# sidward14/gan-lab

Hardware: AMD Instinct MI355X
Metric: images/sec (G+D step), StyleGAN 1024^2 bs32/GPU (higher is better)
Workload: dtype f32; 1 GPU; StyleGAN res_samples=1024 FFHQ-shaped synthetic, bs=32/GPU fp32, nonsaturating + R1(lambda=10) + drift, stabilised phase, 1 D-iter + 1 G-iter; global_batch=32, per_gpu_batch=32, parallelism=single

## Files before the change

### gan_lab_amd/_lib.py

```python
import ctypes
import os
import subprocess

import torch

_HERE = os.path.dirname(os.path.abspath(__file__))
CSRC = os.path.join(_HERE, 'csrc')
SO_PATH = os.path.join(CSRC, os.path.basename(os.environ.get('GANLAB_HIP_LIB', '') or 'libganlab_hip.so'))

_c_int, _c_ll, _c_f, _c_p, _c_sz, _c_u64 = (ctypes.c_int, ctypes.c_longlong, ctypes.c_float, ctypes.c_void_p,
                                             ctypes.c_size_t, ctypes.c_uint64)
_c_d = ctypes.c_double

ACT_NONE, ACT_LRELU = 0, 1
PACK_FWD, PACK_DGRAD = 0, 1


class ConvGeom(ctypes.Structure):
    _fields_ = [('N', _c_int), ('Cin', _c_int), ('Hin', _c_int), ('Win', _c_int),
                ('Cout', _c_int), ('ks', _c_int), ('pad', _c_int), ('up', _c_int), ('pool', _c_int)]


_GP = ctypes.POINTER(ConvGeom)

# ... 42 lines not shown
    'ganlab_conv_splitk_plan': (_c_int, [_GP, _c_int]),
    'ganlab_conv_fwd_splitk_f32': (_c_int, [_c_p, _c_p, _c_p, _c_p, _GP, _c_f, _c_int, _c_f, _c_p, _c_sz, _c_p]),
    'ganlab_conv_dgrad_splitk_f32': (_c_int, [_c_p, _c_p, _c_p, _GP, _c_p, _c_sz, _c_p]),
    'ganlab_conv_dgrad_mask_supported': (_c_int, [_GP]),
    'ganlab_conv_dgrad_mask_f32': (_c_int, [_c_p, _c_p, _c_p, _c_p, _GP, _c_f, _c_p]),
    'ganlab_conv_act_bwd_fused_supported': (_c_int, [_GP]),
    'ganlab_conv_dgrad_act_f32': (_c_int, [_c_p, _c_p, _c_p, _c_p, _GP, _c_f, _c_p]),
    'ganlab_conv_fwd_mask_f32': (_c_int, [_c_p, _c_p, _c_p, _c_p, _GP, _c_f, _c_p]),
    'ganlab_conv_wgrad_act_f32': (_c_int, [_c_p, _c_p, _c_p, _c_p, _c_p, _GP, _c_f, _c_f, _c_f, _c_p, _c_sz, _c_p]),
    'ganlab_conv_wgrad_workspace': (_c_sz, [_GP]),
    'ganlab_conv_wgrad_f32': (_c_int, [_c_p, _c_p, _c_p, _GP, _c_f, _c_p, _c_sz, _c_p]),
    'ganlab_conv_s2_supported': (_c_int, [_GP]),
    'ganlab_conv_s2_pack_f32': (_c_ll, [_c_p, _c_p, _c_int, _c_int, _c_int, _c_int, _c_f, _c_p]),
    'ganlab_conv_s2_fwd_f32': (_c_int, [_c_p, _c_p, _c_p, _c_p, _GP, _c_f, _c_int, _c_f, _c_p]),
    'ganlab_conv_s2_dgrad_f32': (_c_int, [_c_p, _c_p, _c_p, _GP, _c_p]),
    'ganlab_conv_s2_wgrad_workspace': (_c_sz, [_GP]),
    'ganlab_conv_s2_wgrad_f32': (_c_int, [_c_p, _c_p, _c_p, _GP, _c_f, _c_p, _c_sz, _c_p]),
    'ganlab_conv_bf16_supported': (_c_int, [_GP]),
    'ganlab_conv_pack_bf16': (_c_ll, [_c_p, _c_p, _c_int, _c_int, _c_int, _c_f, _c_p]),
    'ganlab_conv_fwd_bf16': (_c_int, [_c_p, _c_p, _c_p, _c_p, _GP, _c_f, _c_int, _c_f, _c_p]),
    'ganlab_conv_dgrad_bf16': (_c_int, [_c_p, _c_p, _c_p, _GP, _c_p]),
    'ganlab_conv_bf16_splitk_plan': (_c_int, [_GP, _c_int]),
    'ganlab_conv_fwd_bf16_splitk': (_c_int, [_c_p, _c_p, _c_p, _c_p, _GP, _c_f, _c_int, _c_f, _c_p, _c_sz, _c_p]),
    'ganlab_conv_dgrad_bf16_splitk': (_c_int, [_c_p, _c_p, _c_p, _GP, _c_p, _c_sz, _c_p]),
    'ganlab_conv_wgrad_bf16_workspace': (_c_sz, [_GP]),
    'ganlab_conv_wgrad_bf16': (_c_int, [_c_p, _c_p, _c_p, _GP, _c_f, _c_p, _c_sz, _c_p]),
    'ganlab_conv_x3_supported': (_c_int, [_GP, _c_int]),
    'ganlab_conv_x3_pack': (_c_ll, [_c_p, _c_p, _c_int, _c_int, _c_int, _c_f, _c_p]),
    'ganlab_conv_fwd_x3': (_c_int, [_c_p, _c_p, _c_p, _c_p, _GP, _c_f, _c_int, _c_f, _c_p]),
    'ganlab_conv_dgrad_x3': (_c_int, [_c_p, _c_p, _c_p, _GP, _c_p]),
    'ganlab_conv_dgrad_mask_x3': (_c_int, [_c_p, _c_p, _c_p, _c_p, _GP, _c_f, _c_p]),
    'ganlab_conv_fwd_aff_x3': (_c_int, [_c_p, _c_p, _c_p, _c_p, _c_p, _c_p, _GP, _c_f, _c_int, _c_f, _c_p]),
    'ganlab_conv_fwd_aff_tail_x3_chunks': (_c_int, [_GP]),
    'ganlab_conv_s2_x3_supported': (_c_int, [_GP, _c_int]),
    'ganlab_conv_s2_x3_pack': (_c_ll, [_c_p, _c_p, _c_int, _c_int, _c_int, _c_f, _c_p]),
    'ganlab_conv_s2_fwd_x3': (_c_int, [_c_p, _c_p, _c_p, _c_p, _GP, _c_f, _c_int, _c_f, _c_p]),
    'ganlab_conv_s2_fwd_aff_x3': (_c_int, [_c_p, _c_p, _c_p, _c_p, _c_p, _c_p, _GP, _c_f, _c_int, _c_f, _c_p]),
    'ganlab_conv_s2_dgrad_x3': (_c_int, [_c_p, _c_p, _c_p, _GP, _c_p]),
    'ganlab_conv_s2_down_x3_supported': (_c_int, [_GP, _c_int]),
    'ganlab_conv_s2_down_x3_pack': (_c_ll, [_c_p, _c_p, _c_int, _c_int, _c_int, _c_f, _c_p]),
    'ganlab_conv_s2_down_fwd_x3': (_c_int, [_c_p, _c_p, _c_p, _c_p, _GP, _c_f, _c_int, _c_f, _c_p]),
    'ganlab_conv_s2_down_dgrad_x3': (_c_int, [_c_p, _c_p, _c_p, _GP, _c_p]),
    'ganlab_conv_wgrad_x3_supported': (_c_int, [_GP]),
    'ganlab_conv_wgrad_x3_workspace': (_c_sz, [_GP]),
    'ganlab_conv_wgrad_x3': (_c_int, [_c_p, _c_p, _c_p, _c_p, _c_p, _GP, _c_f, _c_p, _c_sz, _c_p]),
    'ganlab_conv_s2_wgrad_x3_supported': (_c_int, [_GP]),
    'ganlab_conv_s2_wgrad_x3_workspace': (_c_sz, [_GP]),
    'ganlab_conv_s2_wgrad_x3': (_c_int, [_c_p, _c_p, _c_p, _c_p, _c_p, _GP, _c_f, _c_p, _c_sz, _c_p]),
    'ganlab_conv_fwd_aff_tail_x3': (_c_int, [_c_p, _c_p, _c_p, _c_p, _c_p, _c_p, _c_p, _c_p, _c_p, _c_p, _GP, _c_f, _c_int, _c_f,
                                             _c_f, _c_p, _c_sz, _c_p]),
    'ganlab_mask_bits_supported': (_c_int, [_c_int, _c_int]),
    'ganlab_blur3x3_bits_f32': (_c_int, [_c_p, _c_p, _c_p, _c_ll, _c_int, _c_int, _c_p]),
    'ganlab_blur_act_bwd_bits_f32': (_c_int, [_c_p, _c_p, _c_p, _c_p, _c_int, _c_int, _c_int, _c_int, _c_f, _c_f,
                                              _c_p, _c_sz, _c_p]),
    'ganlab_act_bwd_blur_bits_f32': (_c_int, [_c_p, _c_p, _c_p, _c_p, _c_p, _c_p, _c_int, _c_int, _c_int, _c_int,
                                              _c_f, _c_f, _c_p, _c_sz, _c_p]),
    'ganlab_conv_fwd_blur_supported': (_c_int, [_GP, _c_p, _c_p]),
    'ganlab_conv_fwd_blur_bits_f32': (_c_int, [_c_p, _c_p, _c_p, _c_p, _c_p, _GP, _c_f, _c_f, _c_p]),
    'ganlab_conv_s2_blur_supported': (_c_int, [_GP]),
    'ganlab_conv_s2_blur_workspace': (_c_sz, [_GP]),
    'ganlab_conv_s2_fwd_blur_tail_f32': (_c_int, [_c_p, _c_p, _c_p, _c_p, _c_p, _c_p, _c_p, _c_p, _c_p, _c_p, _GP, _c_f, _c_int,
                                                  _c_f, _c_f, _c_p, _c_sz, _c_p]),
    'ganlab_conv_s2_dgrad_blur_act_bits_f32': (_c_int, [_c_p, _c_p, _c_p, _c_p, _c_p, _GP, _c_f, _c_f, _c_p, _c_sz, _c_p]),
    'ganlab_conv_dgrad_rgb_sums_supported': (_c_int, [_GP, _c_int]),
    'ganlab_conv_dgrad_rgb_sums_workspace': (_c_sz, [_GP]),
    'ganlab_conv_dgrad_rgb_sums_f32': (_c_int, [_c_p, _c_p, _c_p, _c_p, _c_p, _c_p, _GP, _c_int, _c_f, _c_f, _c_f, _c_int, _c_int,
# ... 290 lines not shown
```

### gan_lab_amd/csrc/common.h

```cpp
#pragma once
#include <hip/hip_runtime.h>
#include <stdint.h>

#include "../../include/ganlab_hip.h"

typedef float f32x4 __attribute__((ext_vector_type(4)));

static thread_local int gl_launch_status = GANLAB_OK;
extern thread_local const void* gl_last_kernel_fn;
extern thread_local unsigned gl_last_grid;
#define GL_LAUNCH_RING 16
extern thread_local const void* gl_ring_fn[GL_LAUNCH_RING];
extern thread_local unsigned gl_ring_grid[GL_LAUNCH_RING];
extern thread_local unsigned long long gl_launch_count;
#define GL_LAUNCH(k, grid, ...)                                                  \
  do {                                                                           \
    (void)hipGetLastError();                                                     \
    const dim3 gl_grid_ = (grid);                                                \
    gl_last_kernel_fn = reinterpret_cast<const void*>(k);                        \
    gl_last_grid = gl_grid_.x * gl_grid_.y * gl_grid_.z;                         \
    gl_ring_fn[gl_launch_count % GL_LAUNCH_RING] = gl_last_kernel_fn;            \
    gl_ring_grid[gl_launch_count % GL_LAUNCH_RING] = gl_last_grid;               \
    ++gl_launch_count;                                                           \
    hipLaunchKernelGGL(k, gl_grid_, __VA_ARGS__);                                \
// ... 70 lines not shown
    const float w = ci < Cin ? wp[(long long)ci * Cout_p + co] : 0.f;
    a.x += w * xv[ci].x; a.y += w * xv[ci].y; a.z += w * xv[ci].z; a.w += w * xv[ci].w;
  }
  return a;
}

struct gl_bf16x3 { __bf16 h, m, l; };
__device__ __forceinline__ gl_bf16x3 gl_split3(float v) {
  const __bf16 h = (__bf16)v;
  const float r1 = v - (float)h;
  const __bf16 m = (__bf16)r1;
  return gl_bf16x3{h, m, (__bf16)(r1 - (float)m)};
}

__device__ __forceinline__ void gl_x3_pack_position(const float* __restrict__ w9, bool flip, float scale, __bf16* __restrict__ out,
                                                    int CI, int ci, int co) {
  const int steps = CI / 32 * 9;
  const int ct = co >> 6, col = co & 63, c = ci >> 5, half = (ci >> 4) & 1, g = (ci >> 3) & 1, j = ci & 7;
#pragma unroll
  for (int t = 0; t < 9; ++t) {
    const int s = t < 8 ? (half ? 5 : 0) + (t >> 1) : 4;
    const int hi = t < 8 ? (t & 1) : half;
    const int kg = hi * 2 + g;
    float v = w9[flip ? 8 - t : t] * scale;
    asm volatile("" : "+v"(v));
    const gl_bf16x3 p = gl_split3(v);
    __bf16* base = out + (((long long)ct * steps + c * 9 + s) * (3 * 4 * 64)) * 8;
    base[((0 * 4 + kg) * 64 + col) * 8 + j] = p.h;
    base[((1 * 4 + kg) * 64 + col) * 8 + j] = p.m;
    base[((2 * 4 + kg) * 64 + col) * 8 + j] = p.l;
  }
}

__device__ __forceinline__ void gl_x3_up_pack_position(const float* __restrict__ w9, int up, float scale, __bf16* __restrict__ out,
                                                       int CI, int CO, int ci, int co) {
  const int nsteps = CI / 8;
  const bool c32 = (CO & 63) != 0;
  const int ct = c32 ? co >> 5 : co >> 6, j = ci & 7;
#pragma unroll
  for (int py = 0; py < 2; ++py)
#pragma unroll
    for (int px = 0; px < 2; ++px)
#pragma unroll
      for (int ty = 0; ty < 2; ++ty)
#pragma unroll
        for (int tx = 0; tx < 2; ++tx) {
          float v = 0.f;
#pragma unroll
          for (int ky = 0; ky < 3; ++ky)
#pragma unroll
            for (int kx = 0; kx < 3; ++kx) {
              const int ry = up ? ky : 2 - ky, rx = up ? kx : 2 - kx;
              const bool iny = py == 0 ? (ty == 0 ? ry == 0 : ry >= 1) : (ty == 0 ? ry <= 1 : ry == 2);
              const bool inx = px == 0 ? (tx == 0 ? rx == 0 : rx >= 1) : (tx == 0 ? rx <= 1 : rx == 2);
              if (iny && inx) v += w9[ky * 3 + kx];
            }
          v = v * (up ? scale : 0.25f * scale);
          asm volatile("" : "+v"(v));
          const gl_bf16x3 p = gl_split3(v);
          __bf16* base = out + (((c32 ? (long long)ct : (long long)ct * 2 + py) * nsteps + (ci >> 3)) * (3 * 4 * 128)) * 8;
          const int col = c32 ? py * 32 + (co & 31) : co & 63;
          const int kgq = ty * 2 + tx;
          base[((0 * 4 + kgq) * 128 + px * 64 + col) * 8 + j] = p.h;
          base[((1 * 4 + kgq) * 128 + px * 64 + col) * 8 + j] = p.m;
          base[((2 * 4 + kgq) * 128 + px * 64 + col) * 8 + j] = p.l;
        }
// ... 58 lines not shown
```

### gan_lab_amd/csrc/pack.hip

```cpp
#include "common.h"

namespace {

constexpr int round_up_c(int v, int m) { return (v + m - 1) / m * m; }

__global__ __launch_bounds__(256) void pack_many_kernel(const ganlab_pack_desc* __restrict__ descs, int n_desc) {
  int lo = 0, hi = n_desc - 1;
  const long long b = blockIdx.x;
  while (lo < hi) {
    const int mid = (lo + hi + 1) >> 1;
    if (descs[mid].block0 <= b) lo = mid; else hi = mid - 1;
  }
  const ganlab_pack_desc d = descs[lo];
  const long long e = (b - d.block0) * 256 + threadIdx.x;
  const float* w = d.src;
  if (d.kind == GANLAB_PACKKIND_PLAIN) {
    const int KK = d.ks * d.ks, dgrad = d.mode == GANLAB_PACK_DGRAD;
    const int rows = dgrad ? d.Cout : d.Cin, cols = dgrad ? d.Cin : d.Cout;
    const int rows_p = round_up_c(rows, d.ks == 1 ? 32 : 16), cols_p = round_up_c(cols, 64);
    const long long plane = (long long)rows_p * cols_p;
    if (e >= plane) return;
    const int col = (int)(e % cols_p), row = (int)(e / cols_p);
    const bool in = row < rows && col < cols;
    const int co = dgrad ? row : col, ci = dgrad ? col : row;
// ... 21 lines not shown
      float v = 0.f;
#pragma unroll
      for (int ky = 0; ky < 3; ++ky)
#pragma unroll
        for (int kx = 0; kx < 3; ++kx) v += gl_comb_s2(d.up, a, ky) * gl_comb_s2(d.up, bb, kx) * k9[ky * 3 + kx];
      out[tap * plane] = v * d.scale;
    }
  } else if (d.kind == GANLAB_PACKKIND_X3 && d.ks == 4) {
    const int up = d.up;
    const int CO = up ? d.Cout : d.Cin, CI = up ? d.Cin : d.Cout;
    if (e >= (long long)CO * CI) return;
    int ci, co;
    if ((CO & 63) == 0) {
      const int col = (int)(e & 63);
      const long long t = e >> 6;
      ci = (int)(t % CI);
      co = (int)(t / CI) * 64 + col;
    } else {
      co = (int)(e % CO);
      ci = (int)(e / CO);
    }
    const float* w9 = up ? w + ((long long)co * d.Cin + ci) * 9 : w + ((long long)ci * d.Cin + co) * 9;
    gl_x3_up_pack_position(w9, up, d.scale, reinterpret_cast<__bf16*>(d.dst), CI, CO, ci, co);
  } else if (d.kind == GANLAB_PACKKIND_X3 && d.ks == 5) {
    const int up = d.up;
    const int CO = up ? d.Cin : d.Cout, CI = up ? d.Cout : d.Cin;
    if (e >= (long long)CO * CI) return;
    const int col = (int)(e & 127);
    const long long t = e >> 7;
    const int ci = (int)(t % CI), ct = (int)(t / CI);
    const int co = ct * 128 + col;
    const float* w9 = up ? w + ((long long)ci * d.Cin + co) * 9 : w + ((long long)co * d.Cin + ci) * 9;
    gl_x3_down_pack_position(w9, up, d.scale, reinterpret_cast<__bf16*>(d.dst), CI, ci, co);
  } else if (d.kind == GANLAB_PACKKIND_X3) {
    const bool dg = d.mode == GANLAB_PACK_DGRAD;
    const int CO = dg ? d.Cin : d.Cout, CI = dg ? d.Cout : d.Cin;
    if (e >= (long long)CO * CI) return;
    const int col = (int)(e & 63);
    const long long t = e >> 6;
    const int ci = (int)(t % CI), ct = (int)(t / CI);
    const int co = ct * 64 + col;
    const float* w9 = dg ? w + ((long long)ci * d.Cin + co) * 9 : w + ((long long)co * d.Cin + ci) * 9;
    gl_x3_pack_position(w9, dg, d.scale, reinterpret_cast<__bf16*>(d.dst), CI, ci, co);
  } else {
    const int dg = d.mode == GANLAB_PACK_DGRAD;
    const int CO = dg ? d.Cin : d.Cout;
    if (e >= d.total / 9) return;
    const int j = (int)(e & 7);
    long long t = e >> 3;
    const int co = (int)(t % CO);
    t /= CO;
    const int kg = (int)(t & 3);
    const int chunk = (int)(t >> 2);
    const int ci = chunk * 32 + kg * 8 + j;
    const float* ws = dg ? w + ((long long)ci * d.Cin + co) * 9 : w + ((long long)co * d.Cin + ci) * 9;
    __bf16* out = reinterpret_cast<__bf16*>(d.dst);
#pragma unroll
    for (int tap = 0; tap < 9; ++tap)
      out[((((long long)chunk * 9 + tap) * 4 + kg) * CO + co) * 8 + j] = (__bf16)(ws[dg ? 8 - tap : tap] * d.scale);
  }
}

}

extern "C" {

// ... 10 lines not shown
```

### gan_lab_amd/ops.py

```python
import ctypes
import os

import numpy as np

import torch
from torch.autograd import Function
from torch.autograd.function import once_differentiable

from . import _lib
from ._lib import ACT_LRELU, ACT_NONE, PACK_DGRAD, PACK_FWD, ConvGeom, check
from ._ops.core import (
    _p, _RAW_STREAM, _GET_DEVICE, _st, _c, _inplace, _same_numel, _gpu_device, _new, _ct, _aligned16, _nchw, _row_workspace,
    _INPUT_GRAD_ONLY, input_grad_only, _want_param_grads, _NO_GRAD_TOWARDS, no_grad_towards, _wants_input_grad, _DIRECT, _SINK,
    _TAKEN, direct_grads_enabled, direct_param_grads, _sink, _take, _sunk)
from ._ops.metrics import (
    SWD_DESC, _swd_planes, swd_down, swd_band, swd_gather, swd_stats, swd_project, _SWD_WS, _swd_workspace, swd_sort, swd_distance,
    swd_positions, swd_directions, PRDC_MAX_K, _prdc_rows, _prdc_vector, prdc_norms, prdc_knn, prdc_cross, MOMENTS_MAX_DIM,
    _accumulator, moments_accum, kid_rowsums, PPL_MAX_DIM, PPL_MODES, PPL_SAMPLINGS, PPL_RECORD, check_ppl_epsilon, ppl_endpoints,
    row_sqdist, trimmed_mean, MSSSIM_LEVELS, _msssim_images, msssim_workspace, msssim_level, msssim_finish,
    SPECTRUM_MIN_RES, SPECTRUM_MAX_RES, SPECTRUM_WINDOWS, _spectrum_size, spectrum_scratch_bytes, _spectrum_alloc,
    spectrum_workspace, spectrum_scratch, spectrum_feed, spectrum_finish)
from ._ops.optim import (
    SN_EPS, SnTable, sn_refresh, sn_backward, ortho_plan, OrthoTable, ortho_apply, lerp_rows, _adam_operands, adam_step,
    adam_step_dev, set_step_scalars, ewma_step, EwmaTable, ewma_many)
# ... 131 lines not shown
        _PACK_CACHE.clear()
        _PACK_TABLES.clear()
        _PACK_RANGES.clear()
        return
    for r in ranges:
        _PACK_RANGES[(int(r[0]), int(r[1]))] = _PACK_SERIAL[0]


def pack_generation():
    return _PACK_GEN[0]


_ALL_ADDRESSES = (0, 1 << 62)


def mark_packs_stale():
    if _PACK_RANGES:
        bump_weight_epoch(list(_PACK_RANGES.keys()))
    elif _PACK_CACHE:
        bump_weight_epoch([_ALL_ADDRESSES])


def _pack_one(e):
    L = _lib.lib()
    kind, cout, cin, ks, mode, up, scale, total = e.desc
    if kind == _KIND_S2:
        rc = L.ganlab_conv_s2_pack_f32(_p(e.w), _p(e.out), cout, cin, up, mode, scale, _st())
    elif kind == _KIND_BF16:
        rc = L.ganlab_conv_pack_bf16(_p(e.w), e.out.data_ptr(), cout, cin, mode, scale, _st())
    elif kind == _KIND_X3 and ks == 4:
        rc = L.ganlab_conv_s2_x3_pack(_p(e.w), e.out.data_ptr(), cout, cin, up, scale, _st())
    elif kind == _KIND_X3 and ks == 5:
        rc = L.ganlab_conv_s2_down_x3_pack(_p(e.w), e.out.data_ptr(), cout, cin, up, scale, _st())
    elif kind == _KIND_X3:
        rc = L.ganlab_conv_x3_pack(_p(e.w), e.out.data_ptr(), cout, cin, mode, scale, _st())
    else:
        rc = L.ganlab_conv_pack_f32(_p(e.w), _p(e.out), cout, cin, ks, mode, scale, _st())
    if rc != total:
        raise _lib.GanlabLibraryError(f're-pack failed ({rc} != {total})')


def _stale_range(e):
    for r, ser in _PACK_RANGES.items():
        if ser > e.serial and r[0] <= e.ptr < r[1]:
            return r
    return None


def _repack_range(r):
    L = _lib.lib()
    ser = _PACK_RANGES[r]
    items = [(k, e) for k, e in _PACK_CACHE.items() if r[0] <= e.ptr < r[1] and e.serial < ser]
    keys = tuple(k for k, _ in items)
    tab = _PACK_TABLES.get(r)
    if (tab is None or tab[0] != keys) and torch.cuda.is_current_stream_capturing():
        for _, e in items:
            _pack_one(e)
            e.serial = _PACK_SERIAL[0]
        return
    if tab is None or tab[0] != keys:
        arr = (_lib.PackDesc * len(items))()
        blocks = 0
        for i, (_, e) in enumerate(items):
            kind, cout, cin, ks, mode, up, scale, total = e.desc
            d = arr[i]
            d.src, d.dst = e.w.data_ptr(), e.out.data_ptr()
# ... 133 lines not shown
    L = _lib.lib()
    ws = torch.empty((L.ganlab_conv_s2_wgrad_x3_workspace(g.ref()) + 3) // 4, dtype=torch.float32, device=x.device)
    check(L.ganlab_conv_s2_wgrad_x3(_p(gy), _p(x), _p(s_), _p(t_), _p(gw), g.ref(), scale, _p(ws), ws.numel() * 4, _st()),
          'conv_s2_wgrad_x3')
    return gw


def x3_s2_down_ok(g, dgrad=False):
    if not _X3[0] or not g.s2:
        return False
    if (g.up if dgrad else g.pool) != 1:
        return False
    co = g.Cin if dgrad else g.Cout
    hl, wl = (g.Hin, g.Win) if dgrad else (g.Hin // 2, g.Win // 2)
    if g.N * (hl // 8) * (wl // 16) * (co // 128) < _X3_MIN_TILES:
        return False
    return bool(_lib.lib().ganlab_conv_s2_down_x3_supported(g.ref(), 1 if dgrad else 0))


def _packed_x3_any(name, tag, w, sel, scale, ks):
    key = (w.data_ptr(), w._version, tuple(w.shape), sel, float(scale), tag)
    hit = _pack_lookup(key)
    if hit is not None:
        return hit
    cout, cin = w.shape[0], w.shape[1]
    pack = getattr(_lib.lib(), 'ganlab_' + name)
    n = pack(None, None, cout, cin, sel, scale, None)
    if n <= 0:
        raise _lib.GanlabLibraryError(f'{name} size query failed ({n}) for weight {tuple(w.shape)}')
    out = torch.empty((n,), dtype=torch.bfloat16, device=w.device)
    rc = pack(_p(w), out.data_ptr(), cout, cin, sel, scale, _st())
    if rc != n:
        raise _lib.GanlabLibraryError(f'{name} failed ({rc})')
    mode, up = (sel, 0) if ks == 3 else (0, sel)
    return _pack_store(key, w, out, (_KIND_X3, cout, cin, ks, mode, up, float(scale), int(n)))


def _packed_x3_s2_down(w, up, scale):
    return _packed_x3_any('conv_s2_down_x3_pack', 'x3s2d', w, int(up), scale, 5)


def _packed_x3_s2(w, up, scale):
    return _packed_x3_any('conv_s2_x3_pack', 'x3s2', w, int(up), scale, 4)


def _packed_x3(w, mode, scale):
    return _packed_x3_any('conv_x3_pack', 'x3', w, mode, scale, 3)


_OBSERVER = [None]


def set_launch_observer(fn):
    prev = _OBSERVER[0]
    _OBSERVER[0] = fn
    return prev


def conv_flops(g):
    if g.s2:
        lo_h, lo_w = (g.Hin, g.Win) if g.up else (g.Ho, g.Wo)
        return 2.0 * 16 * g.Cin * g.Cout * lo_h * lo_w * g.N
    if g.bf is not None:
        return 2.0 * g.ks * g.ks * g.Cin * g.Cout * g.bf.Hin * g.bf.Win * g.N
    return 2.0 * g.ks * g.ks * g.Cin * g.Cout * g.Ho * g.Wo * g.N


def _note(kind, g):
    if _OBSERVER[0] is not None:
        _OBSERVER[0](kind, g)


def k_conv_fwd(x, w, bias, g, scale, bias_scale=1.0, act=ACT_NONE, slope=0.2):
    x, w = _c(x, 'conv input'), _c(w, 'conv weight')
    assert tuple(x.shape) == g.in_shape, (tuple(x.shape), g.in_shape)
    assert tuple(w.shape) == (g.Cout, g.Cin, g.ks, g.ks), (tuple(w.shape), g.Cout, g.Cin, g.ks)
    _note('fwd', g)
    if bias is not None:
        bias = _c(bias, 'bias')
        assert bias.numel() == g.Cout
# ... 11 lines not shown
                                                slope, _p(ws), ws.numel() * 4, _st()), 'conv_fwd_bf16_splitk')
            return y
        check(L.ganlab_conv_fwd_bf16(_p(xin), wp.data_ptr(), _p(bias), _p(y), ctypes.byref(geom), bias_scale,
                                     act, slope, _st()), 'conv_fwd_bf16')
        return y
    if x3_s2_down_ok(g):
        check(_lib.lib().ganlab_conv_s2_down_fwd_x3(_p(x), _packed_x3_s2_down(w, 0, scale).data_ptr(), _p(bias), _p(y), g.ref(),
                                                    bias_scale, act, slope, _st()), 'conv_s2_down_fwd_x3')
        return y
    if x3_s2_ok(g):
        check(_lib.lib().ganlab_conv_s2_fwd_x3(_p(x), _packed_x3_s2(w, 1, scale).data_ptr(), _p(bias), _p(y), g.ref(), bias_scale,
                                               act, slope, _st()), 'conv_s2_fwd_x3')
        return y
    if g.s2:
        wp = _packed(w, PACK_FWD, scale, s2_up=g.up)
        check(_lib.lib().ganlab_conv_s2_fwd_f32(_p(x), _p(wp), _p(bias), _p(y), g.ref(), bias_scale, act, slope,
                                                _st()), 'conv_s2_fwd')
        return y
    if g.ks == 1 and g.Hin == 1 and g.Win == 1 and g.N <= 64 and g.Cin >= 2048 and g.Cin % 128 == 0:
        g2 = Geom(1, g.Cout, g.Cin // 128, 128, g.N, 1, 0)
        obs = set_launch_observer(None)
        try:
            y = k_conv_wgrad(x.view(g2.out_shape), w.view(g2.in_shape), g2, scale).view(g.out_shape)
        finally:
            set_launch_observer(obs)
        if bias is not None or act != ACT_NONE:
            y = k_bias_act(y, bias, None, None, bias_scale, act, slope)
        return y
    L = _lib.lib()
    if x3_ok(g):
        check(L.ganlab_conv_fwd_x3(_p(x), _packed_x3(w, PACK_FWD, scale).data_ptr(), _p(bias), _p(y), g.ref(), bias_scale, act,
                                   slope, _st()), 'conv_fwd_x3')
        return y
    wp = _packed(w, PACK_FWD, scale)
    split = 0 if g.up else L.ganlab_conv_splitk_plan(g.ref(), 0)
    if split >= 2:
        ws = torch.empty((split,) + tuple(y.shape), dtype=torch.float32, device=x.device)
        check(L.ganlab_conv_fwd_splitk_f32(_p(x), _p(wp), _p(bias), _p(y), g.ref(), bias_scale, act, slope, _p(ws),
                                           ws.numel() * 4, _st()), 'conv_fwd_splitk')
        return y
    check(L.ganlab_conv_fwd_f32(_p(x), _p(wp), _p(bias), _p(y), g.ref(), bias_scale, act, slope, _st()), 'conv_fwd')
    return y


def k_conv_dgrad(gy, w, g, scale):
    gy, w = _c(gy, 'conv grad_out'), _c(w, 'conv weight')
    assert tuple(gy.shape) == g.out_shape, (tuple(gy.shape), g.out_shape)
    _note('dgrad', g)
    if g.bf is not None:
        wp = _packed_bf16(w, PACK_DGRAD, scale)
        L = _lib.lib()

        def run(geom, out):
            split = L.ganlab_conv_bf16_splitk_plan(ctypes.byref(geom), 1)
            if split >= 2:
                m = 2 if geom.up else 1
                ws = torch.empty((split * geom.N * geom.Cin * geom.Hin * m * geom.Win * m,), dtype=torch.float32,
                                 device=gy.device)
                check(L.ganlab_conv_dgrad_bf16_splitk(_p(gy), wp.data_ptr(), _p(out), ctypes.byref(geom), _p(ws),
                                                      ws.numel() * 4, _st()), 'conv_dgrad_bf16_splitk')
            else:
                check(L.ganlab_conv_dgrad_bf16(_p(gy), wp.data_ptr(), _p(out), ctypes.byref(geom), _st()), 'conv_dgrad_bf16')
            return out
        if g.bf_fused is not None:
            return run(g.bf_fused, _new(g.in_shape, gy))
        gxv = run(g.bf, _new((g.N, g.Cin, g.bf.Hin, g.bf.Win), gy))
        return k_pool2(gxv, 1.0) if g.up else gxv
    if x3_s2_down_ok(g, True):
        gx = _new(g.in_shape, gy)
        check(_lib.lib().ganlab_conv_s2_down_dgrad_x3(_p(gy), _packed_x3_s2_down(w, 1, scale).data_ptr(), _p(gx), g.ref(), _st()),
              'conv_s2_down_dgrad_x3')
        return gx
    if x3_s2_ok(g, True):
        gx = _new(g.in_shape, gy)
        check(_lib.lib().ganlab_conv_s2_dgrad_x3(_p(gy), _packed_x3_s2(w, 0, scale).data_ptr(), _p(gx), g.ref(), _st()),
              'conv_s2_dgrad_x3')
        return gx
    if g.s2:
        wp = _packed(w, PACK_DGRAD, scale, s2_up=g.up)
        gx = _new(g.in_shape, gy)
        check(_lib.lib().ganlab_conv_s2_dgrad_f32(_p(gy), _p(wp), _p(gx), g.ref(), _st()), 'conv_s2_dgrad')
        return gx
    if x3_ok(g, True):
        gx = _new(g.in_shape, gy)
        check(_lib.lib().ganlab_conv_dgrad_x3(_p(gy), _packed_x3(w, PACK_DGRAD, scale).data_ptr(), _p(gx), g.ref(), _st()),
              'conv_dgrad_x3')
        return gx
    wp = _packed(w, PACK_DGRAD, scale)
    hv, wv = (2 * g.Hin, 2 * g.Win) if g.up else (g.Hin, g.Win)
    gxv = _new((g.N, g.Cin, hv, wv), gy)
    split = 0 if g.up else _lib.lib().ganlab_conv_splitk_plan(g.ref(), 1)
    if split >= 2:
        ws = torch.empty((split,) + tuple(gxv.shape), dtype=torch.float32, device=gy.device)
        check(_lib.lib().ganlab_conv_dgrad_splitk_f32(_p(gy), _p(wp), _p(gxv), g.ref(), _p(ws), ws.numel() * 4, _st()),
              'conv_dgrad_splitk')
        return gxv
    check(_lib.lib().ganlab_conv_dgrad_f32(_p(gy), _p(wp), _p(gxv), g.ref(), _st()), 'conv_dgrad')
    if g.up:
        return k_pool2(gxv, 1.0)
    return gxv


def conv_dgrad_mask_ok(g):
    return g.bf is None and not g.s2 and not g.up and bool(_lib.lib().ganlab_conv_dgrad_mask_supported(g.ref()))


def k_conv_dgrad_mask(gy, w, x, g, scale, slope):
    gy, w, x = _c(gy, 'conv grad_out'), _c(w, 'conv weight'), _c(x, 'conv input')
    assert tuple(gy.shape) == g.out_shape and tuple(x.shape) == g.in_shape
    _note('dgrad', g)
    gx = torch.empty_like(x)
    if x3_ok(g, True):
        check(_lib.lib().ganlab_conv_dgrad_mask_x3(_p(gy), _packed_x3(w, PACK_DGRAD, scale).data_ptr(), _p(x), _p(gx), g.ref(),
                                                   slope, _st()), 'conv_dgrad_mask_x3')
        return gx
    check(_lib.lib().ganlab_conv_dgrad_mask_f32(_p(gy), _p(_packed(w, PACK_DGRAD, scale)), _p(x), _p(gx), g.ref(), slope,
                                                _st()), 'conv_dgrad_mask')
    return gx

# ... 2495 lines not shown
```

### include/ganlab_hip.h

```cpp
#ifndef GANLAB_HIP_H
#define GANLAB_HIP_H

#include <stddef.h>
#include <stdint.h>

#ifdef __cplusplus
extern "C" {
#endif

#define GANLAB_OK 0
#define GANLAB_EINVAL (-1)
#define GANLAB_EWORKSPACE (-2)
#define GANLAB_ELAUNCH (-3)
#define GANLAB_EUNSUPPORTED (-4)

#define GANLAB_ACT_NONE 0
#define GANLAB_ACT_LRELU 1

#define GANLAB_PACK_FWD 0
#define GANLAB_PACK_DGRAD 1

int ganlab_abi_version(void);

int ganlab_last_launch(char* name, int cap, unsigned* grid);
// ... 51 lines not shown
int ganlab_conv_s2_fwd_f32(const float* x, const float* wp, const float* bias, float* y,
                           const ganlab_conv_geom* g, float bias_scale, int act, float slope, void* stream);
int ganlab_conv_s2_dgrad_f32(const float* gy, const float* wp, float* gx, const ganlab_conv_geom* g,
                             void* stream);
size_t ganlab_conv_s2_wgrad_workspace(const ganlab_conv_geom* g);
int ganlab_conv_s2_wgrad_f32(const float* gy, const float* x, float* gw, const ganlab_conv_geom* g,
                             float scale, void* workspace, size_t workspace_bytes, void* stream);

int ganlab_conv_bf16_supported(const ganlab_conv_geom* g);
long long ganlab_conv_pack_bf16(const float* w, void* out, int Cout, int Cin, int mode, float scale, void* stream);
int ganlab_conv_fwd_bf16(const float* x, const void* wp, const float* bias, float* y, const ganlab_conv_geom* g,
                         float bias_scale, int act, float slope, void* stream);
int ganlab_conv_dgrad_bf16(const float* gy, const void* wp, float* gx, const ganlab_conv_geom* g, void* stream);
int ganlab_conv_bf16_splitk_plan(const ganlab_conv_geom* g, int dgrad);
int ganlab_conv_fwd_bf16_splitk(const float* x, const void* wp, const float* bias, float* y, const ganlab_conv_geom* g,
                                float bias_scale, int act, float slope, void* workspace, size_t workspace_bytes,
                                void* stream);
int ganlab_conv_dgrad_bf16_splitk(const float* gy, const void* wp, float* gx, const ganlab_conv_geom* g, void* workspace,
                                  size_t workspace_bytes, void* stream);
size_t ganlab_conv_wgrad_bf16_workspace(const ganlab_conv_geom* g);
int ganlab_conv_wgrad_bf16(const float* gy, const float* x, float* gw, const ganlab_conv_geom* g, float scale,
                           void* workspace, size_t workspace_bytes, void* stream);

int ganlab_conv_x3_supported(const ganlab_conv_geom* g, int dgrad);
long long ganlab_conv_x3_pack(const float* w, void* out, int Cout, int Cin, int mode, float scale, void* stream);
int ganlab_conv_fwd_x3(const float* x, const void* wp, const float* bias, float* y, const ganlab_conv_geom* g,
                       float bias_scale, int act, float slope, void* stream);
int ganlab_conv_dgrad_x3(const float* gy, const void* wp, float* gx, const ganlab_conv_geom* g, void* stream);
int ganlab_conv_dgrad_mask_x3(const float* gy, const void* wp, const float* x, float* gx, const ganlab_conv_geom* g,
                              float slope, void* stream);
int ganlab_conv_fwd_aff_x3(const float* x, const void* wp, const float* aff_s, const float* aff_t, const float* bias,
                           float* y, const ganlab_conv_geom* g, float bias_scale, int act, float slope, void* stream);
int ganlab_conv_fwd_aff_tail_x3_chunks(const ganlab_conv_geom* g);
int ganlab_conv_s2_x3_supported(const ganlab_conv_geom* g, int dgrad);
long long ganlab_conv_s2_x3_pack(const float* w, void* out, int Cout, int Cin, int up, float scale, void* stream);
int ganlab_conv_s2_fwd_x3(const float* x, const void* wp, const float* bias, float* y, const ganlab_conv_geom* g,
                          float bias_scale, int act, float slope, void* stream);
int ganlab_conv_s2_fwd_aff_x3(const float* x, const void* wp, const float* aff_s, const float* aff_t, const float* bias,
                              float* y, const ganlab_conv_geom* g, float bias_scale, int act, float slope, void* stream);
int ganlab_conv_s2_dgrad_x3(const float* gy, const void* wp, float* gx, const ganlab_conv_geom* g, void* stream);
int ganlab_conv_s2_down_x3_supported(const ganlab_conv_geom* g, int dgrad);
long long ganlab_conv_s2_down_x3_pack(const float* w, void* out, int Cout, int Cin, int up, float scale, void* stream);
int ganlab_conv_s2_down_fwd_x3(const float* x, const void* wp, const float* bias, float* y, const ganlab_conv_geom* g,
                               float bias_scale, int act, float slope, void* stream);
int ganlab_conv_s2_down_dgrad_x3(const float* gy, const void* wp, float* gx, const ganlab_conv_geom* g, void* stream);
int ganlab_conv_wgrad_x3_supported(const ganlab_conv_geom* g);
size_t ganlab_conv_wgrad_x3_workspace(const ganlab_conv_geom* g);
int ganlab_conv_wgrad_x3(const float* gy, const float* x, const float* aff_s, const float* aff_t, float* gw,
                         const ganlab_conv_geom* g, float scale, void* workspace, size_t workspace_bytes, void* stream);
int ganlab_conv_s2_wgrad_x3_supported(const ganlab_conv_geom* g);
size_t ganlab_conv_s2_wgrad_x3_workspace(const ganlab_conv_geom* g);
int ganlab_conv_s2_wgrad_x3(const float* gy, const float* x, const float* aff_s, const float* aff_t, float* gw,
                            const ganlab_conv_geom* g, float scale, void* workspace, size_t workspace_bytes, void* stream);
int ganlab_conv_fwd_aff_tail_x3(const float* x, const void* wp, const float* aff_s, const float* aff_t, const float* bias,
                                const float* noise, const float* noise_w, float* y, float* mean, float* rstd,
                                const ganlab_conv_geom* g, float bias_scale, int act, float slope, float eps, void* workspace,
                                size_t workspace_bytes, void* stream);

int ganlab_blur3x3_f32(const float* x, float* y, long long planes, int H, int W, void* stream);
int ganlab_up2_f32(const float* x, float* y, long long planes, int H, int W, float scale, void* stream);
int ganlab_pool2_f32(const float* x, float* y, long long planes, int Hout, int Wout, float scale,
                     void* stream);
int ganlab_resample2d_f32(const float* x, float* y, const int* iy, const float* wy, const int* ix, const float* wx,
                          long long planes, int Hi, int Wi, int Ho, int Wo, int Ty, int Tx, void* stream);

int ganlab_bias_act_f32(const float* x, const float* bias, const float* noise, const float* noise_w,
// ... 463 lines not shown
```

Before: 169.6 images/sec.

## Add rolling-row-ring bf16x3 MFMA kernel for 16-channel 3x3 convs

Adds a dedicated forward/dgrad kernel for 3x3 pad-1 convolutions with 16 input and 16 output channels, as used at the highest StyleGAN resolutions. Input rows are streamed into a six-slot LDS ring buffer split into bf16 hi/mid/lo planes, and the next rows are loaded while MFMAs run on the current ones. Weights stay in registers, and work is split across blocks into row strips per column tile. The aim is to replace generic kernels that underuse MFMA tiles at these narrow channel counts. It adds a new weight pack format and a dispatch path that is taken only when alignment and shape conditions hold.

```diff
diff --git a/gan_lab_amd/_lib.py b/gan_lab_amd/_lib.py
--- a/gan_lab_amd/_lib.py
+++ b/gan_lab_amd/_lib.py
@@ -98,6 +98,10 @@
     'ganlab_conv_dgrad_mask_x3': (_c_int, [_c_p, _c_p, _c_p, _c_p, _GP, _c_f, _c_p]),
     'ganlab_conv_fwd_aff_x3': (_c_int, [_c_p, _c_p, _c_p, _c_p, _c_p, _c_p, _GP, _c_f, _c_int, _c_f, _c_p]),
     'ganlab_conv_fwd_aff_tail_x3_chunks': (_c_int, [_GP]),
+    'ganlab_conv_x3_roll_supported': (_c_int, [_GP, _c_p, _c_p]),
+    'ganlab_conv_x3_roll_pack': (_c_ll, [_c_p, _c_p, _c_int, _c_int, _c_int, _c_f, _c_p]),
+    'ganlab_conv_fwd_x3_roll': (_c_int, [_c_p, _c_p, _c_p, _c_p, _GP, _c_f, _c_int, _c_f, _c_p]),
+    'ganlab_conv_dgrad_x3_roll': (_c_int, [_c_p, _c_p, _c_p, _GP, _c_p]),
     'ganlab_conv_s2_x3_supported': (_c_int, [_GP, _c_int]),
     'ganlab_conv_s2_x3_pack': (_c_ll, [_c_p, _c_p, _c_int, _c_int, _c_int, _c_f, _c_p]),
     'ganlab_conv_s2_fwd_x3': (_c_int, [_c_p, _c_p, _c_p, _c_p, _GP, _c_f, _c_int, _c_f, _c_p]),
diff --git a/gan_lab_amd/csrc/common.h b/gan_lab_amd/csrc/common.h
--- a/gan_lab_amd/csrc/common.h
+++ b/gan_lab_amd/csrc/common.h
@@ -126,6 +126,22 @@
   }
 }
 
+constexpr int GL_X3_ROLL_ELEMS = 3 * 5 * 4 * 16 * 8;
+__device__ __forceinline__ void gl_x3_roll_pack_position(const float* __restrict__ w9, bool flip, float scale, __bf16* __restrict__ out,
+                                                         int ci, int co) {
+  const int g = ci >> 3, j = ci & 7;
+#pragma unroll
+  for (int t = 0; t < 10; ++t) {
+    float v = (t < 9 && w9 != nullptr) ? w9[flip ? 8 - t : t] * scale : 0.f;
+    asm volatile("" : "+v"(v));
+    const gl_bf16x3 p = gl_split3(v);
+    const int at = ((((t >> 1) * 4) + (t & 1) * 2 + g) * 16 + co) * 8 + j;
+    out[at] = p.h;
+    out[at + GL_X3_ROLL_ELEMS / 3] = p.m;
+    out[at + 2 * (GL_X3_ROLL_ELEMS / 3)] = p.l;
+  }
+}
+
 __device__ __forceinline__ void gl_x3_up_pack_position(const float* __restrict__ w9, int up, float scale, __bf16* __restrict__ out,
                                                        int CI, int CO, int ci, int co) {
   const int nsteps = CI / 8;
diff --git a/gan_lab_amd/csrc/conv_x3_roll.hip b/gan_lab_amd/csrc/conv_x3_roll.hip
--- /dev/null
+++ b/gan_lab_amd/csrc/conv_x3_roll.hip
@@ -0,0 +1,214 @@
+#include "x3_common.h"
+
+namespace {
+
+constexpr int XR_TW = 64, XR_SLOTS = 6, XR_Q = 18;
+constexpr int XR_PLANE = 66, XR_HALF = 208;
+constexpr int XR_ROW = XR_HALF + 3 * XR_PLANE;
+constexpr int XR_RING = XR_SLOTS * XR_ROW;
+constexpr int XR_ITEMS_PER_WAVE = 2 * 4 * XR_Q / 4;
+constexpr int XR_OOB = (int)0x80000000;
+
+struct XRArgs {
+  const float* x;
+  const u32x4* wp;
+  const float* bias;
+  float* y;
+  int N, H, W;
+  int cols, strips, spu;
+  float bias_scale, slope;
+  int act;
+};
+
+__global__ void x3_roll_pack_kernel(const float* __restrict__ w, __bf16* __restrict__ out, int Cout, int Cin, int mode, float scale) {
+  const bool dg = mode == GANLAB_PACK_DGRAD;
+  const int CO = dg ? Cin : Cout, CI = dg ? Cout : Cin;
+  const int e = threadIdx.x;
+  const int co = e & 15, ci = e >> 4;
+  const float* w9 = dg ? w + ((long long)ci * Cin + co) * 9 : w + ((long long)co * Cin + ci) * 9;
+  gl_x3_roll_pack_position((ci < CI && co < CO) ? w9 : nullptr, dg, scale, out, ci, co);
+}
+
+__device__ __forceinline__ f32x4 xr_mfma(const u32x4& a, const u32x4& b, const f32x4& c) {
+  return __builtin_amdgcn_mfma_f32_16x16x32_bf16(__builtin_bit_cast(bf16x8, a), __builtin_bit_cast(bf16x8, b), c, 0, 0, 0);
+}
+
+__global__ __launch_bounds__(256, 3) void conv_x3_roll_plain_kernel(XRArgs p) {
+  __shared__ __attribute__((aligned(16))) u32x4 ring[XR_RING];
+  const int tid = threadIdx.x, lane = tid & 63, w = tid >> 6;
+  const int co = lane & 15, kk = lane >> 4;
+  const bool hi = kk >= 2;
+  int bid = gl_xcd_remap(blockIdx.x, gridDim.x);
+  const int txi = bid % p.cols;
+  bid /= p.cols;
+  const int syi = bid % p.strips;
+  const int n0 = bid / p.strips;
+  const int nh = 2 * min(p.spu, p.H / 4 - syi * p.spu);
+  const int ox0 = txi * XR_TW, Y0 = syi * p.spu * 4;
+  const int plane = p.H * p.W, W4 = p.W * 4;
+
+  const bool stager = lane < XR_ITEMS_PER_WAVE;
+  const int se = w * XR_ITEMS_PER_WAVE + (stager ? lane : 0);
+  const int sq = se % XR_Q, st_ = se / XR_Q, cq = st_ & 3, sk = st_ >> 2;
+  const int svx = ox0 - 4 + 4 * sq;
+  const int gb = (stager && (unsigned)svx < (unsigned)p.W) ? (cq * 4 * plane + svx) * 4 : XR_OOB;
+  const int px_lo = !stager ? 4 : (sq == 0 ? 3 : 0), px_hi = sq == XR_Q - 1 ? 0 : 3;
+  const int st_lane = 2 * ((cq >> 1) * XR_HALF + 4 * sq - 3) + (cq & 1);
+  const int rot = sq >> 1;
+
+  u32x4 wreg[3][5];
+#pragma unroll
+  for (int pl = 0; pl < 3; ++pl)
+#pragma unroll
+    for (int s = 0; s < 5; ++s) wreg[pl][s] = p.wp[((pl * 5 + s) * 4 + kk) * 16 + co];
+  const float bv = p.bias != nullptr ? p.bias[co] * p.bias_scale : 0.f;
+
+  const __amdgpu_buffer_rsrc_t rs_in = __builtin_amdgcn_make_buffer_rsrc(
+      const_cast<float*>(p.x + (long long)n0 * 16 * plane), 0, (unsigned)(16 * plane * 4), 0x00020000);
+  const __amdgpu_buffer_rsrc_t rs_out =
+      __builtin_amdgcn_make_buffer_rsrc(p.y + (long long)n0 * 16 * plane, 0, (unsigned)(16 * plane * 4), 0x00020000);
+  const int vo_lane = (co * plane + ox0 + w * 16 + kk * 4) * 4;
+
+  f32x4 xr[4];
+  auto load_rows = [&](int r0, bool on) {
+    const int vy = Y0 - 1 + r0 + sk;
+    const bool ok = on && gb != XR_OOB && (unsigned)vy < (unsigned)p.H;
+#pragma unroll
+    for (int c = 0; c < 4; ++c) {
+      const u32x4 v = __builtin_amdgcn_raw_buffer_load_b128(rs_in, ok ? gb + c * plane * 4 + vy * W4 : XR_OOB, 0, 0);
+      xr[c] = __builtin_bit_cast(f32x4, v);
+    }
+  };
+  u32x2* ring8 = reinterpret_cast<u32x2*>(ring);
+  auto store_rows = [&](int slot0) {
+    const int base = 2 * (slot0 + sk) * XR_ROW + st_lane;
+#pragma unroll
+    for (int jj = 0; jj < 4; ++jj) {
+      const int j = (jj + rot) & 3;
+      auto pick = [&](const f32x4& v) { return j == 0 ? v[0] : j == 1 ? v[1] : j == 2 ? v[2] : v[3]; };
+      u32x2 h, m, l;
+      x3_split4(f32x4{pick(xr[0]), pick(xr[1]), pick(xr[2]), pick(xr[3])}, h, m, l);
+      if (j >= px_lo && j <= px_hi) {
+        ring8[base + 2 * j] = h;
+        ring8[base + 2 * j + 2 * XR_PLANE] = m;
+        ring8[base + 2 * j + 4 * XR_PLANE] = l;
+      }
+    }
+  };
+
+  load_rows(0, true);
+  store_rows(0);
+  load_rows(2, true);
+  store_rows(2);
+  load_rows(4, true);
+  __syncthreads();
+
+  f32x4 accH[2], accS[2];
+#pragma unroll
+  for (int r2 = 0; r2 < 2; ++r2) accH[r2] = accS[r2] = f32x4{0.f, 0.f, 0.f, 0.f};
+  const int a_lane = (kk & 1) * XR_HALF + w * 16 + co;
+  int s0 = 0;
+  for (int h = 0; h < nh; ++h) {
+    int rowb[4];
+#pragma unroll
+    for (int j = 0; j < 4; ++j) rowb[j] = (s0 + j >= XR_SLOTS ? s0 + j - XR_SLOTS : s0 + j) * XR_ROW + a_lane;
+#pragma unroll
+    for (int s = 0; s < 5; ++s) {
+#pragma unroll
+      for (int r2 = 0; r2 < 2; ++r2) {
+        int at;
+        if (s == 0) at = rowb[r2] + (hi ? 1 : 0);
+        else if (s == 1) at = hi ? rowb[r2 + 1] : rowb[r2] + 2;
+        else if (s == 2) at = rowb[r2 + 1] + (hi ? 2 : 1);
+        else if (s == 3) at = rowb[r2 + 2] + (hi ? 1 : 0);
+        else at = rowb[r2 + 2] + 2;
+        const u32x4 ah = ring[at], am = ring[at + XR_PLANE], al = ring[at + 2 * XR_PLANE];
+        accH[r2] = xr_mfma(ah, wreg[0][s], accH[r2]);
+        accS[r2] = xr_mfma(ah, wreg[1][s], accS[r2]);
+        accS[r2] = xr_mfma(am, wreg[0][s], accS[r2]);
+        accS[r2] = xr_mfma(am, wreg[1][s], accS[r2]);
+        accS[r2] = xr_mfma(ah, wreg[2][s], accS[r2]);
+        accS[r2] = xr_mfma(al, wreg[0][s], accS[r2]);
+      }
+      if (s == 1) store_rows(s0 >= 2 ? s0 - 2 : s0 + 4);
+      if (s == 2) load_rows(2 * h + 6, h + 2 < nh);
+    }
+#pragma unroll
+    for (int r2 = 0; r2 < 2; ++r2) {
+      const int row = Y0 + 2 * h + r2;
+      const f32x4 v = accH[r2] + accS[r2];
+      u32x4 o;
+#pragma unroll
+      for (int r = 0; r < 4; ++r) {
+        float t = v[r] + bv;
+        if (p.act == GANLAB_ACT_LRELU) t = gl_lrelu(t, p.slope);
+        o[r] = __float_as_uint(t);
+      }
+      __builtin_amdgcn_raw_buffer_store_b128(o, rs_out, vo_lane + row * W4, 0, 0);
+      accH[r2] = accS[r2] = f32x4{0.f, 0.f, 0.f, 0.f};
+    }
+    s0 = s0 == 4 ? 0 : s0 + 2;
+    __syncthreads();
+  }
+}
+
+long long xr_plan(XRArgs& a, int N, int H, int W) {
+  a.cols = W / XR_TW;
+  const int steps = H / 4;
+  const long long cols = (long long)a.cols * N;
+  int k = 1;
+  while (k < steps && cols * k < 4096 && (steps + k) / (k + 1) >= 8) ++k;
+  a.spu = (steps + k - 1) / k;
+  a.strips = (steps + a.spu - 1) / a.spu;
+  return cols * a.strips;
+}
+
+bool xr_ok(const ganlab_conv_geom* g, const void* x, const void* y) {
+  if (g == nullptr || g->ks != 3 || g->pad != 1 || g->up || g->pool || g->N <= 0 || g->Cin != 16 || g->Cout != 16) return false;
+  if (g->Hin <= 0 || g->Win <= 0 || g->Win % XR_TW != 0 || g->Hin % 4 != 0) return false;
+  if (16LL * g->Hin * g->Win * 4 >= 0x7fffffffLL) return false;
+  XRArgs a{};
+  const long long grid = xr_plan(a, g->N, g->Hin, g->Win);
+  if (grid <= 0 || grid > 0x7fffffffLL) return false;
+  return (reinterpret_cast<uintptr_t>(x) & 15) == 0 && (reinterpret_cast<uintptr_t>(y) & 15) == 0;
+}
+
+int xr_launch(const float* x, const void* wp, const float* bias, float* y, const ganlab_conv_geom* g, float bias_scale, int act,
+              float slope, hipStream_t st) {
+  if (x == nullptr || wp == nullptr || y == nullptr) return GANLAB_EINVAL;
+  if (!xr_ok(g, x, y) || (reinterpret_cast<uintptr_t>(wp) & 15) != 0) return GANLAB_EUNSUPPORTED;
+  XRArgs a{};
+  a.x = x; a.wp = reinterpret_cast<const u32x4*>(wp); a.bias = bias; a.y = y;
+  a.N = g->N; a.H = g->Hin; a.W = g->Win;
+  a.bias_scale = bias_scale; a.slope = slope; a.act = act;
+  const long long grid = xr_plan(a, a.N, a.H, a.W);
+  GL_LAUNCH(conv_x3_roll_plain_kernel, dim3((unsigned)grid), dim3(256), 0, st, a);
+  return GL_CHECK_LAUNCH();
+}
+
+}
+
+extern "C" {
+
+int ganlab_conv_x3_roll_supported(const ganlab_conv_geom* g, const void* x, const void* y) { return xr_ok(g, x, y) ? 1 : 0; }
+
+long long ganlab_conv_x3_roll_pack(const float* w, void* out, int Cout, int Cin, int mode, float scale, void* stream) {
+  if (Cout <= 0 || Cin <= 0 || Cout > 16 || Cin > 16 || (mode != GANLAB_PACK_FWD && mode != GANLAB_PACK_DGRAD)) return GANLAB_EINVAL;
+  const long long n = GL_X3_ROLL_ELEMS;
+  if (out == nullptr) return n;
+  if (w == nullptr) return GANLAB_EINVAL;
+  GL_LAUNCH(x3_roll_pack_kernel, dim3(1), dim3(256), 0, gl_stream(stream), w, reinterpret_cast<__bf16*>(out), Cout, Cin, mode, scale);
+  const int st = GL_CHECK_LAUNCH();
+  return st != GANLAB_OK ? st : n;
+}
+
+int ganlab_conv_fwd_x3_roll(const float* x, const void* wp, const float* bias, float* y, const ganlab_conv_geom* g,
+                            float bias_scale, int act, float slope, void* stream) {
+  return xr_launch(x, wp, bias, y, g, bias_scale, act, slope, gl_stream(stream));
+}
+
+int ganlab_conv_dgrad_x3_roll(const float* gy, const void* wp, float* gx, const ganlab_conv_geom* g, void* stream) {
+  return xr_launch(gy, wp, nullptr, gx, g, 1.f, GANLAB_ACT_NONE, 0.f, gl_stream(stream));
+}
+
+}
diff --git a/gan_lab_amd/csrc/pack.hip b/gan_lab_amd/csrc/pack.hip
--- a/gan_lab_amd/csrc/pack.hip
+++ b/gan_lab_amd/csrc/pack.hip
@@ -77,6 +77,13 @@
     const int co = ct * 128 + col;
     const float* w9 = up ? w + ((long long)ci * d.Cin + co) * 9 : w + ((long long)co * d.Cin + ci) * 9;
     gl_x3_down_pack_position(w9, up, d.scale, reinterpret_cast<__bf16*>(d.dst), CI, ci, co);
+  } else if (d.kind == GANLAB_PACKKIND_X3 && d.ks == 6) {
+    if (e >= 256) return;
+    const bool dg = d.mode == GANLAB_PACK_DGRAD;
+    const int CO = dg ? d.Cin : d.Cout, CI = dg ? d.Cout : d.Cin;
+    const int co = (int)(e & 15), ci = (int)(e >> 4);
+    const float* w9 = dg ? w + ((long long)ci * d.Cin + co) * 9 : w + ((long long)co * d.Cin + ci) * 9;
+    gl_x3_roll_pack_position((ci < CI && co < CO) ? w9 : nullptr, dg, d.scale, reinterpret_cast<__bf16*>(d.dst), ci, co);
   } else if (d.kind == GANLAB_PACKKIND_X3) {
     const bool dg = d.mode == GANLAB_PACK_DGRAD;
     const int CO = dg ? d.Cin : d.Cout, CI = dg ? d.Cout : d.Cin;
diff --git a/gan_lab_amd/ops.py b/gan_lab_amd/ops.py
--- a/gan_lab_amd/ops.py
+++ b/gan_lab_amd/ops.py
@@ -187,6 +187,8 @@
         rc = L.ganlab_conv_s2_x3_pack(_p(e.w), e.out.data_ptr(), cout, cin, up, scale, _st())
     elif kind == _KIND_X3 and ks == 5:
         rc = L.ganlab_conv_s2_down_x3_pack(_p(e.w), e.out.data_ptr(), cout, cin, up, scale, _st())
+    elif kind == _KIND_X3 and ks == 6:
+        rc = L.ganlab_conv_x3_roll_pack(_p(e.w), e.out.data_ptr(), cout, cin, mode, scale, _st())
     elif kind == _KIND_X3:
         rc = L.ganlab_conv_x3_pack(_p(e.w), e.out.data_ptr(), cout, cin, mode, scale, _st())
     else:
@@ -386,7 +388,7 @@
     rc = pack(_p(w), out.data_ptr(), cout, cin, sel, scale, _st())
     if rc != n:
         raise _lib.GanlabLibraryError(f'{name} failed ({rc})')
-    mode, up = (sel, 0) if ks == 3 else (0, sel)
+    mode, up = (sel, 0) if ks in (3, 6) else (0, sel)
     return _pack_store(key, w, out, (_KIND_X3, cout, cin, ks, mode, up, float(scale), int(n)))
 
 
@@ -400,6 +402,16 @@
 
 def _packed_x3(w, mode, scale):
     return _packed_x3_any('conv_x3_pack', 'x3', w, mode, scale, 3)
+
+
+def x3_roll_ok(g, x, y):
+    if not _X3[0] or g.Cin != 16 or g.Cout != 16 or g.ks != 3 or g.pad != 1 or g.bf is not None or g.s2 or g.up or g.pool:
+        return False
+    return bool(_lib.lib().ganlab_conv_x3_roll_supported(g.ref(), _p(x), _p(y)))
+
+
+def _packed_x3_roll(w, mode, scale):
+    return _packed_x3_any('conv_x3_roll_pack', 'x3roll', w, mode, scale, 6)
 
 
 _OBSERVER = [None]
@@ -477,6 +489,10 @@
         check(L.ganlab_conv_fwd_x3(_p(x), _packed_x3(w, PACK_FWD, scale).data_ptr(), _p(bias), _p(y), g.ref(), bias_scale, act,
                                    slope, _st()), 'conv_fwd_x3')
         return y
+    if x3_roll_ok(g, x, y):
+        check(L.ganlab_conv_fwd_x3_roll(_p(x), _packed_x3_roll(w, PACK_FWD, scale).data_ptr(), _p(bias), _p(y), g.ref(), bias_scale,
+                                        act, slope, _st()), 'conv_fwd_x3_roll')
+        return y
     wp = _packed(w, PACK_FWD, scale)
     split = 0 if g.up else L.ganlab_conv_splitk_plan(g.ref(), 0)
     if split >= 2:
@@ -530,6 +546,11 @@
         gx = _new(g.in_shape, gy)
         check(_lib.lib().ganlab_conv_dgrad_x3(_p(gy), _packed_x3(w, PACK_DGRAD, scale).data_ptr(), _p(gx), g.ref(), _st()),
               'conv_dgrad_x3')
+        return gx
+    if x3_roll_ok(g, gy, None):
+        gx = _new(g.in_shape, gy)
+        check(_lib.lib().ganlab_conv_dgrad_x3_roll(_p(gy), _packed_x3_roll(w, PACK_DGRAD, scale).data_ptr(), _p(gx), g.ref(),
+                                                   _st()), 'conv_dgrad_x3_roll')
         return gx
     wp = _packed(w, PACK_DGRAD, scale)
     hv, wv = (2 * g.Hin, 2 * g.Win) if g.up else (g.Hin, g.Win)
diff --git a/include/ganlab_hip.h b/include/ganlab_hip.h
--- a/include/ganlab_hip.h
+++ b/include/ganlab_hip.h
@@ -107,6 +107,11 @@
 int ganlab_conv_fwd_aff_x3(const float* x, const void* wp, const float* aff_s, const float* aff_t, const float* bias,
                            float* y, const ganlab_conv_geom* g, float bias_scale, int act, float slope, void* stream);
 int ganlab_conv_fwd_aff_tail_x3_chunks(const ganlab_conv_geom* g);
+int ganlab_conv_x3_roll_supported(const ganlab_conv_geom* g, const void* x, const void* y);
+long long ganlab_conv_x3_roll_pack(const float* w, void* out, int Cout, int Cin, int mode, float scale, void* stream);
+int ganlab_conv_fwd_x3_roll(const float* x, const void* wp, const float* bias, float* y, const ganlab_conv_geom* g,
+                            float bias_scale, int act, float slope, void* stream);
+int ganlab_conv_dgrad_x3_roll(const float* gy, const void* wp, float* gx, const ganlab_conv_geom* g, void* stream);
 int ganlab_conv_s2_x3_supported(const ganlab_conv_geom* g, int dgrad);
 long long ganlab_conv_s2_x3_pack(const float* w, void* out, int Cout, int Cin, int up, float scale, void* stream);
 int ganlab_conv_s2_fwd_x3(const float* x, const void* wp, const float* bias, float* y, const ganlab_conv_geom* g,
```

Result: no change. 169.4 images/sec, median of 2 (-0.1%).
